# stm233/image-compression-for-machine

Measured on AMD Instinct MI355X. Metric: images/sec (256x256) cnn-hyperprior (WACNN) training step, higher is better.
Workload: dtype f32; 1 GPU; cnn (WACNN N=192 M=320) train step, lambda=0.0067 MSE, batch 16/GPU synthetic 256x256, Adam lr 1e-4 + aux Adam, clip 1.0; global_batch=16, parallelism=dp1

## Files before the change

image-compression-for-machine_amd/csrc/winattn_mfma.hip:

```cpp
#include "icm_common.h"

namespace icm {

struct WaDesc;

struct WmDesc {
  const float* qkv;
  const float* table;
  float* out;
  const float* dout;
  float* dqkv;
  float* dtable_ws;
  int N, C, H, W, heads, shift, nwx, nwy;
  float scale;
};

#define WM_WS 8
#define WM_T 64
#define WM_TS 65
#define WM_NTAB 225

__device__ __forceinline__ int wm_region(int s, int L, int shift) { return s < L - WM_WS ? 0 : (s < L - shift ? 1 : 2); }

__device__ __forceinline__ void wm_token(const WmDesc& d, int wy, int wx, int t, int& pix, int& lab) {
  const int r = t >> 3, c = t & 7;
  const int sy = wy * WM_WS + r, sx = wx * WM_WS + c;
  int oy = sy + d.shift, ox = sx + d.shift;
  if (oy >= d.H) oy -= d.H;
  if (ox >= d.W) ox -= d.W;
  pix = oy * d.W + ox;
  lab = d.shift > 0 ? wm_region(sy, d.H, d.shift) * 3 + wm_region(sx, d.W, d.shift) : 0;
}

__device__ __forceinline__ int wm_row(int r) { return (r & 3) + 8 * (r >> 2); }
__device__ __forceinline__ int wm_relidx(int i, int j) {
  return ((i >> 3) - (j >> 3) + WM_WS - 1) * (2 * WM_WS - 1) + ((i & 7) - (j & 7) + WM_WS - 1);
}

template <int HD>
__device__ __forceinline__ void wm_tok_tok(const float* __restrict__ rowT, const float* __restrict__ colT, int lane,
                                           f32x16 (&acc)[2][2]) {
  const int l31 = lane & 31, h = lane >> 5;
#pragma unroll
  for (int x = 0; x < 2; ++x)
#pragma unroll
    for (int y = 0; y < 2; ++y)
#pragma unroll
      for (int r = 0; r < 16; ++r) acc[x][y][r] = 0.0f;
#pragma unroll
  for (int ks = 0; ks < HD / 2; ++ks) {
    const int off = (2 * ks + h) * WM_TS + l31;
    const float a0 = rowT[off], a1 = rowT[off + 32], b0 = colT[off], b1 = colT[off + 32];
    acc[0][0] = __builtin_amdgcn_mfma_f32_32x32x2f32(a0, b0, acc[0][0], 0, 0, 0);
    acc[0][1] = __builtin_amdgcn_mfma_f32_32x32x2f32(a0, b1, acc[0][1], 0, 0, 0);
    acc[1][0] = __builtin_amdgcn_mfma_f32_32x32x2f32(a1, b0, acc[1][0], 0, 0, 0);
    acc[1][1] = __builtin_amdgcn_mfma_f32_32x32x2f32(a1, b1, acc[1][1], 0, 0, 0);
  }
}

template <int HD, int ND>
__device__ __forceinline__ void wm_ch_tok(const float* __restrict__ chT, const f32x16 (&M)[2][2], int lane,
                                          f32x16 (&o)[ND][2]) {
  const int l31 = lane & 31, h = lane >> 5;
#pragma unroll
  for (int dt = 0; dt < ND; ++dt)
#pragma unroll
    for (int y = 0; y < 2; ++y)
#pragma unroll
      for (int r = 0; r < 16; ++r) o[dt][y][r] = 0.0f;
#pragma unroll
  for (int x = 0; x < 2; ++x)
#pragma unroll
    for (int r = 0; r < 16; ++r) {
      const int tok = x * 32 + wm_row(r) + 4 * h;
#pragma unroll
      for (int dt = 0; dt < ND; ++dt) {
        const int dd = min(dt * 32 + l31, HD - 1);
        const float a = chT[dd * WM_TS + tok];
        o[dt][0] = __builtin_amdgcn_mfma_f32_32x32x2f32(a, M[x][0][r], o[dt][0], 0, 0, 0);
        o[dt][1] = __builtin_amdgcn_mfma_f32_32x32x2f32(a, M[x][1][r], o[dt][1], 0, 0, 0);
      }
    }
}

template <int HD, int ND>
__device__ __forceinline__ void wm_store(float* __restrict__ base, long long HW, const int (&pix)[2], int lane,
                                         const f32x16 (&o)[ND][2], float mul) {
  const int h = lane >> 5;
#pragma unroll
  for (int dt = 0; dt < ND; ++dt)
#pragma unroll
    for (int r = 0; r < 16; ++r) {
      const int dd = dt * 32 + wm_row(r) + 4 * h;
      if (dd < HD) {
        base[(long long)dd * HW + pix[0]] = o[dt][0][r] * mul;
        base[(long long)dd * HW + pix[1]] = o[dt][1][r] * mul;
      }
    }
}

template <int HD, int NS>
__device__ __forceinline__ void wm_load_all(const float* const (&src)[NS], long long HW, int pix, int lane, float mul0,
                                            float* __restrict__ dst0) {
  float v[NS][HD];
#pragma unroll
  for (int k = 0; k < NS; ++k)
#pragma unroll
    for (int dd = 0; dd < HD; ++dd) v[k][dd] = src[k][(long long)dd * HW + pix];
#pragma unroll
  for (int k = 0; k < NS; ++k)
#pragma unroll
    for (int dd = 0; dd < HD; ++dd) dst0[(k * HD + dd) * WM_TS + lane] = k == 0 ? v[k][dd] * mul0 : v[k][dd];
}

__device__ __forceinline__ float wm_xhalf(float v) { return __shfl_xor(v, 32, 64); }

__device__ __forceinline__ void wm_softmax_T(f32x16 (&acc)[2][2], const float* __restrict__ bias, const int (&labq)[2],
                                             const unsigned char* __restrict__ labs, bool masked, int lane,
                                             float (&m)[2], float (&linv)[2]) {
  const int l31 = lane & 31, h = lane >> 5;
#pragma unroll
  for (int it = 0; it < 2; ++it) {
    const int i = it * 32 + l31;
    float mx = -3.0e38f;
#pragma unroll
    for (int jt = 0; jt < 2; ++jt)
#pragma unroll
      for (int r = 0; r < 16; ++r) {
        const int j = jt * 32 + wm_row(r) + 4 * h;
        float s = acc[jt][it][r] + bias[wm_relidx(i, j)];
        if (masked && labs[j] != labq[it]) s += -100.0f;
        acc[jt][it][r] = s;
        mx = fmaxf(mx, s);
      }
    mx = fmaxf(mx, wm_xhalf(mx));
    float sum = 0.0f;
#pragma unroll
    for (int jt = 0; jt < 2; ++jt)
#pragma unroll
      for (int r = 0; r < 16; ++r) {
        const float p = expf(acc[jt][it][r] - mx);
        acc[jt][it][r] = p;
        sum += p;
      }
    sum += wm_xhalf(sum);
    const float inv = 1.0f / sum;
#pragma unroll
    for (int jt = 0; jt < 2; ++jt)
#pragma unroll
      for (int r = 0; r < 16; ++r) acc[jt][it][r] *= inv;
    m[it] = mx;
    linv[it] = inv;
  }
}

template <int HD, int NS>
struct WmLds {
  static constexpr int kSlab = HD * WM_TS;
  static constexpr int kFloats = NS * kSlab + 228 + (NS > 3 ? 228 + 3 * WM_T : 0);
};

template <int HD>
__global__ __launch_bounds__(256, 2) void winattn_mfma_fwd_kernel(const WmDesc d) {
  extern __shared__ __attribute__((aligned(16))) float smem[];
  constexpr int ND = (HD + 31) / 32;
  using LDS = WmLds<HD, 3>;
  int* pixs = reinterpret_cast<int*>(smem + 4 * LDS::kFloats);
  unsigned char* labs = reinterpret_cast<unsigned char*>(pixs + WM_T);
  const int tid = threadIdx.x, lane = tid & 63, wave = __builtin_amdgcn_readfirstlane(tid >> 6);
  float* Qt = smem + wave * LDS::kFloats;
  float* Kt = Qt + LDS::kSlab;
  float* Vt = Kt + LDS::kSlab;
  float* bias = Vt + LDS::kSlab;
  int bid = xcd_block_id();
  const int wx = bid % d.nwx; bid /= d.nwx;
  const int wy = bid % d.nwy;
  const int n = bid / d.nwy;
  const long long HW = (long long)d.H * d.W;
  if (tid < WM_T) {
    int px, lb;
    wm_token(d, wy, wx, tid, px, lb);
    pixs[tid] = px;
    labs[tid] = (unsigned char)lb;
  }
  __syncthreads();
  const int l31 = lane & 31;
  const int mypix = pixs[lane];
  const int pix2[2] = {pixs[l31], pixs[32 + l31]};
  const int labq[2] = {labs[l31], labs[32 + l31]};
  const float* base = d.qkv + (long long)n * 3 * d.C * HW;
  const bool masked = d.shift > 0;
  for (int head = wave; head < d.heads; head += 4) {
    {
      const float* const srcs[3] = {base + (long long)(head * HD) * HW, base + (long long)(d.C + head * HD) * HW,
                                    base + (long long)(2 * d.C + head * HD) * HW};
      wm_load_all<HD, 3>(srcs, HW, mypix, lane, d.scale, Qt);
    }
    for (int e = lane; e < WM_NTAB; e += 64) bias[e] = d.table[e * d.heads + head];
    __builtin_amdgcn_s_waitcnt(0);
    __builtin_amdgcn_wave_barrier();
    f32x16 st[2][2];
    wm_tok_tok<HD>(Kt, Qt, lane, st);
    float m[2], linv[2];
    wm_softmax_T(st, bias, labq, labs, masked, lane, m, linv);
    f32x16 o[ND][2];
    wm_ch_tok<HD, ND>(Vt, st, lane, o);
    wm_store<HD, ND>(d.out + ((long long)n * d.C + head * HD) * HW, HW, pix2, lane, o, 1.0f);
    __builtin_amdgcn_s_waitcnt(0);
    __builtin_amdgcn_wave_barrier();
  }
}

template <int HD>
__global__ __launch_bounds__(256, 1) void winattn_mfma_bwd_kernel(const WmDesc d) {
  extern __shared__ __attribute__((aligned(16))) float smem[];
  constexpr int ND = (HD + 31) / 32;
  using LDS = WmLds<HD, 4>;
  int* pixs = reinterpret_cast<int*>(smem + 4 * LDS::kFloats);
  unsigned char* labs = reinterpret_cast<unsigned char*>(pixs + WM_T);
  const int tid = threadIdx.x, lane = tid & 63, wave = __builtin_amdgcn_readfirstlane(tid >> 6);
  float* Qt = smem + wave * LDS::kFloats;
  float* Kt = Qt + LDS::kSlab;
  float* Vt = Kt + LDS::kSlab;
  float* Gt = Vt + LDS::kSlab;
  float* bias = Gt + LDS::kSlab;
  float* dbias = bias + 228;
  float* stat_m = dbias + 228;
  float* stat_l = stat_m + WM_T;
  float* stat_d = stat_l + WM_T;
  int bid = xcd_block_id();
  const int win = bid;
  const int wx = bid % d.nwx; bid /= d.nwx;
  const int wy = bid % d.nwy;
  const int n = bid / d.nwy;
  const long long HW = (long long)d.H * d.W;
  if (tid < WM_T) {
    int px, lb;
    wm_token(d, wy, wx, tid, px, lb);
    pixs[tid] = px;
    labs[tid] = (unsigned char)lb;
  }
  __syncthreads();
  const int l31 = lane & 31, h = lane >> 5;
  const int mypix = pixs[lane];
  const int pix2[2] = {pixs[l31], pixs[32 + l31]};
  const int labq[2] = {labs[l31], labs[32 + l31]};
  const float* base = d.qkv + (long long)n * 3 * d.C * HW;
  float* dbase = d.dqkv + (long long)n * 3 * d.C * HW;
  const bool masked = d.shift > 0;
  for (int head = wave; head < d.heads; head += 4) {
    {
      const float* const srcs[4] = {base + (long long)(head * HD) * HW, base + (long long)(d.C + head * HD) * HW,
                                    base + (long long)(2 * d.C + head * HD) * HW,
                                    d.dout + ((long long)n * d.C + head * HD) * HW};
      wm_load_all<HD, 4>(srcs, HW, mypix, lane, d.scale, Qt);
    }
    for (int e = lane; e < WM_NTAB; e += 64) {
      bias[e] = d.table[e * d.heads + head];
      dbias[e] = 0.0f;
    }
    __builtin_amdgcn_s_waitcnt(0);
    __builtin_amdgcn_wave_barrier();
    {
      f32x16 pt[2][2];
      wm_tok_tok<HD>(Kt, Qt, lane, pt);
      float m[2], linv[2];
      wm_softmax_T(pt, bias, labq, labs, masked, lane, m, linv);
      if (h == 0) {
        stat_m[l31] = m[0]; stat_m[32 + l31] = m[1];
        stat_l[l31] = linv[0]; stat_l[32 + l31] = linv[1];
      }
      f32x16 dpt[2][2];
      wm_tok_tok<HD>(Vt, Gt, lane, dpt);
#pragma unroll
      for (int it = 0; it < 2; ++it) {
        float del = 0.0f;
#pragma unroll
        for (int jt = 0; jt < 2; ++jt)
#pragma unroll
          for (int r = 0; r < 16; ++r) del += pt[jt][it][r] * dpt[jt][it][r];
        del += wm_xhalf(del);
        if (h == 0) stat_d[it * 32 + l31] = del;
#pragma unroll
        for (int jt = 0; jt < 2; ++jt)
#pragma unroll
          for (int r = 0; r < 16; ++r) pt[jt][it][r] *= dpt[jt][it][r] - del;
      }
#pragma unroll
      for (int hh = 0; hh < 2; ++hh) {
        if (h == hh) {
#pragma unroll
          for (int it = 0; it < 2; ++it)
#pragma unroll
            for (int jt = 0; jt < 2; ++jt)
#pragma unroll
              for (int r = 0; r < 16; ++r) {
                const int idx = wm_relidx(it * 32 + l31, jt * 32 + wm_row(r) + 4 * h);
                __hip_atomic_fetch_add(dbias + idx, pt[jt][it][r], __ATOMIC_RELAXED, __HIP_MEMORY_SCOPE_WAVEFRONT);
              }
        }
        __builtin_amdgcn_s_waitcnt(0);
        __builtin_amdgcn_wave_barrier();
      }
      f32x16 o[ND][2];
      wm_ch_tok<HD, ND>(Kt, pt, lane, o);
      wm_store<HD, ND>(dbase + (long long)(head * HD) * HW, HW, pix2, lane, o, d.scale);
    }
    __builtin_amdgcn_s_waitcnt(0);
    __builtin_amdgcn_wave_barrier();
    {
      f32x16 p[2][2];
      wm_tok_tok<HD>(Qt, Kt, lane, p);
#pragma unroll
      for (int it = 0; it < 2; ++it)
#pragma unroll
        for (int r = 0; r < 16; ++r) {
          const int i = it * 32 + wm_row(r) + 4 * h;
          const float mi = stat_m[i], li = stat_l[i];
          const int labi = labs[i];
#pragma unroll
          for (int jt = 0; jt < 2; ++jt) {
            const int j = jt * 32 + l31;
            float s = p[it][jt][r] + bias[wm_relidx(i, j)];
            if (masked && labq[jt] != labi) s += -100.0f;
            p[it][jt][r] = expf(s - mi) * li;
          }
        }
      {
        f32x16 o[ND][2];
        wm_ch_tok<HD, ND>(Gt, p, lane, o);
        wm_store<HD, ND>(dbase + (long long)(2 * d.C + head * HD) * HW, HW, pix2, lane, o, 1.0f);
      }
      f32x16 dp[2][2];
      wm_tok_tok<HD>(Gt, Vt, lane, dp);
#pragma unroll
      for (int it = 0; it < 2; ++it)
#pragma unroll
        for (int r = 0; r < 16; ++r) {
          const float del = stat_d[it * 32 + wm_row(r) + 4 * h];
#pragma unroll
          for (int jt = 0; jt < 2; ++jt) p[it][jt][r] *= dp[it][jt][r] - del;
        }
      f32x16 o[ND][2];
      wm_ch_tok<HD, ND>(Qt, p, lane, o);
      wm_store<HD, ND>(dbase + (long long)(d.C + head * HD) * HW, HW, pix2, lane, o, 1.0f);
    }
    {
      float* slab = d.dtable_ws + ((long long)win * d.heads + head) * WM_NTAB;
      for (int e = lane; e < WM_NTAB; e += 64) slab[e] = dbias[e];
    }
    __builtin_amdgcn_s_waitcnt(0);
    __builtin_amdgcn_wave_barrier();
  }
}

typedef void (*WmFn)(const WmDesc);
static bool wm_pick(int hd, WmFn& f, WmFn& b, size_t& lf, size_t& lb) {
  switch (hd) {
#define C_(n)                                               \
  case n:                                                   \
    f = winattn_mfma_fwd_kernel<n>;                         \
    b = winattn_mfma_bwd_kernel<n>;                         \
    lf = ((size_t)4 * WmLds<n, 3>::kFloats + WM_T + WM_T / 4) * sizeof(float);  \
    lb = ((size_t)4 * WmLds<n, 4>::kFloats + WM_T + WM_T / 4) * sizeof(float);  \
    return true;
    C_(8) C_(16) C_(24) C_(32) C_(48)
#undef C_
    default: return false;
  }
}

static bool wm_fill(WmDesc& d, int N, int C, int H, int W, int heads, int ws, int shift) {
  if (ws != WM_WS || heads <= 0 || C % heads || H % ws || W % ws || shift < 0 || shift >= ws) return false;
  d.N = N; d.C = C; d.H = H; d.W = W; d.heads = heads; d.shift = shift;
  d.nwx = W / ws; d.nwy = H / ws;
  d.scale = 1.0f / sqrtf((float)(C / heads));
  return true;
}

int winattn_mfma_fwd(const float* qkv, const float* table, float* out, int N, int C, int H, int W, int heads, int ws,
                     int shift, hipStream_t stream) {
  WmDesc d{};
  WmFn f, b;
  size_t lf, lb;
  if (!wm_fill(d, N, C, H, W, heads, ws, shift) || !wm_pick(C / heads, f, b, lf, lb)) return -1;
  d.qkv = qkv; d.table = table; d.out = out;
  if (lf > 64 * 1024 && !ensure_max_lds(reinterpret_cast<const void*>(f))) return ICM_ERR_LAUNCH;
  hipLaunchKernelGGL(f, dim3(N * d.nwy * d.nwx), dim3(256), lf, stream, d);
  ICM_CHECK_LAUNCH();
  return ICM_OK;
}

int winattn_mfma_bwd(const float* qkv, const float* table, const float* dout, float* dqkv, float* dtable_ws, int N, int C,
                     int H, int W, int heads, int ws, int shift, hipStream_t stream) {
  WmDesc d{};
  WmFn f, b;
  size_t lf, lb;
  if (!wm_fill(d, N, C, H, W, heads, ws, shift) || !wm_pick(C / heads, f, b, lf, lb)) return -1;
  d.qkv = qkv; d.table = table; d.dout = dout; d.dqkv = dqkv; d.dtable_ws = dtable_ws;
  if (lb > 160 * 1024) return -1;
  if (lb > 64 * 1024 && !ensure_max_lds(reinterpret_cast<const void*>(b))) return ICM_ERR_LAUNCH;
  hipLaunchKernelGGL(b, dim3(N * d.nwy * d.nwx), dim3(256), lb, stream, d);
  ICM_CHECK_LAUNCH();
  return ICM_OK;
}

}

namespace icm {

#define W4_T 16
#define W4_TS 17
#define W4_NTAB 49

struct W4Desc {
  const float* qkv;
  const float* table;
  float* out;
  const float* dout;
  float* dqkv;
  float* dtable_ws;
  int N, C, H, W, heads, shift, ngx, nwy;
  float scale;
};

typedef float f32x4v __attribute__((ext_vector_type(4)));

__device__ __forceinline__ int w4_region(int s, int L, int shift) { return s < L - 4 ? 0 : (s < L - shift ? 1 : 2); }

template <int HD>
__device__ __forceinline__ f32x4v w4_tok_tok(const float* __restrict__ rowT, const float* __restrict__ colT, int lane) {
  const int t = lane & 15, g = lane >> 4;
  f32x4v acc = {0.0f, 0.0f, 0.0f, 0.0f};
#pragma unroll
  for (int ks = 0; ks < HD / 4; ++ks) {
    const int off = (4 * ks + g) * W4_TS + t;
    acc = __builtin_amdgcn_mfma_f32_16x16x4f32(rowT[off], colT[off], acc, 0, 0, 0);
  }
  return acc;
}
template <int HD, int ND>
__device__ __forceinline__ void w4_ch_tok(const float* __restrict__ chT, const f32x4v M, int lane, f32x4v (&o)[ND]) {
  const int t = lane & 15, g = lane >> 4;
#pragma unroll
  for (int dt = 0; dt < ND; ++dt) {
    o[dt] = f32x4v{0.0f, 0.0f, 0.0f, 0.0f};
    const int dd = min(dt * 16 + t, HD - 1);
#pragma unroll
    for (int r = 0; r < 4; ++r)
      o[dt] = __builtin_amdgcn_mfma_f32_16x16x4f32(chT[dd * W4_TS + 4 * g + r], M[r], o[dt], 0, 0, 0);
  }
}
template <int HD, int ND>
__device__ __forceinline__ void w4_store(float* __restrict__ base, long long HW, int pix, int lane, const f32x4v (&o)[ND],
                                         float mul) {
  const int g = lane >> 4;
#pragma unroll
  for (int dt = 0; dt < ND; ++dt)
#pragma unroll
    for (int r = 0; r < 4; ++r) {
      const int dd = dt * 16 + 4 * g + r;
      if (dd < HD) base[(long long)dd * HW + pix] = o[dt][r] * mul;
    }
}
__device__ __forceinline__ float w4_xgroups(float v, bool is_max) {
  const float a = __shfl_xor(v, 16, 64);
  v = is_max ? fmaxf(v, a) : v + a;
  const float b = __shfl_xor(v, 32, 64);
  return is_max ? fmaxf(v, b) : v + b;
}
__device__ __forceinline__ int w4_relidx(int i, int j) { return ((i >> 2) - (j >> 2) + 3) * 7 + ((i & 3) - (j & 3) + 3); }

template <int HD, int NS>
struct W4Lds {
  static constexpr int kSlab = HD * W4_TS;
  static constexpr int kFloats = NS * 4 * kSlab + 52 + (NS > 3 ? 52 + 3 * 64 : 0);
};

template <int HD, int NS>
__device__ __forceinline__ void w4_load_all(const float* const (&src)[NS], long long HW, int pix, int lane, float mul0,
                                            float* __restrict__ dst0) {
  const int w = lane >> 4, t = lane & 15;
  float v[NS][HD];
#pragma unroll
  for (int k = 0; k < NS; ++k)
#pragma unroll
    for (int dd = 0; dd < HD; ++dd) v[k][dd] = src[k][(long long)dd * HW + pix];
#pragma unroll
  for (int k = 0; k < NS; ++k)
#pragma unroll
    for (int dd = 0; dd < HD; ++dd)
      dst0[((k * 4 + w) * HD + dd) * W4_TS + t] = k == 0 ? v[k][dd] * mul0 : v[k][dd];
}

__device__ __forceinline__ void w4_token(const W4Desc& d, int wy, int gx, int w, int t, int& pix, int& lab, bool& valid) {
  const int wx = gx * 4 + w;
  valid = wx * 4 < d.W;
  const int r = t >> 2, c = t & 3;
  const int sy = wy * 4 + r, sx = min(wx, d.W / 4 - 1) * 4 + c;
  int oy = sy + d.shift, ox = sx + d.shift;
  if (oy >= d.H) oy -= d.H;
  if (ox >= d.W) ox -= d.W;
  pix = oy * d.W + ox;
  lab = d.shift > 0 ? w4_region(sy, d.H, d.shift) * 3 + w4_region(sx, d.W, d.shift) : 0;
}

template <int HD>
__global__ __launch_bounds__(256) void winattn_mfma16_fwd_kernel(const W4Desc d) {
  extern __shared__ __attribute__((aligned(16))) float smem[];
  constexpr int ND = (HD + 15) / 16;
  using LDS = W4Lds<HD, 3>;
  const int tid = threadIdx.x, lane = tid & 63, wave = __builtin_amdgcn_readfirstlane(tid >> 6);
  float* slabs = smem + wave * LDS::kFloats;
  float* bias = slabs + 3 * 4 * LDS::kSlab;
  const int wt = blockIdx.x * 4 + wave;
  const int ntask = d.N * d.nwy * d.ngx;
  if (wt >= ntask * d.heads) return;
  const int head = wt % d.heads, task = wt / d.heads;
  const int gx = task % d.ngx;
  const int wy = (task / d.ngx) % d.nwy;
  const int n = task / (d.ngx * d.nwy);
  const long long HW = (long long)d.H * d.W;
  const int t = lane & 15, g = lane >> 4;
  int mypix, mylab;
  bool myvalid;
  w4_token(d, wy, gx, g, t, mypix, mylab, myvalid);
  const float* base = d.qkv + (long long)n * 3 * d.C * HW;
  const bool masked = d.shift > 0;
  {
    {
      const float* const srcs[3] = {base + (long long)(head * HD) * HW, base + (long long)(d.C + head * HD) * HW,
                                    base + (long long)(2 * d.C + head * HD) * HW};
      w4_load_all<HD, 3>(srcs, HW, mypix, lane, d.scale, slabs);
    }
    if (lane < W4_NTAB) bias[lane] = d.table[lane * d.heads + head];
    __builtin_amdgcn_s_waitcnt(0);
    __builtin_amdgcn_wave_barrier();
#pragma unroll 1
    for (int w = 0; w < 4; ++w) {
      int pixw, labq;
      bool validw;
      w4_token(d, wy, gx, w, t, pixw, labq, validw);
      if (!validw) break;
      const float* Qt = slabs + (0 * 4 + w) * LDS::kSlab;
      const float* Kt = slabs + (1 * 4 + w) * LDS::kSlab;
      const float* Vt = slabs + (2 * 4 + w) * LDS::kSlab;
      f32x4v st = w4_tok_tok<HD>(Kt, Qt, lane);
      float mx = -3.0e38f;
#pragma unroll
      for (int r = 0; r < 4; ++r) {
        const int j = 4 * g + r;
        float s = st[r] + bias[w4_relidx(t, j)];
        if (masked) {
          int pj, lj; bool vj;
          w4_token(d, wy, gx, w, j, pj, lj, vj);
          if (lj != labq) s += -100.0f;
        }
        st[r] = s;
        mx = fmaxf(mx, s);
      }
      mx = w4_xgroups(mx, true);
      float sum = 0.0f;
#pragma unroll
      for (int r = 0; r < 4; ++r) { st[r] = expf(st[r] - mx); sum += st[r]; }
      sum = w4_xgroups(sum, false);
      const float inv = 1.0f / sum;
#pragma unroll
      for (int r = 0; r < 4; ++r) st[r] *= inv;
      f32x4v o[ND];
      w4_ch_tok<HD, ND>(Vt, st, lane, o);
      w4_store<HD, ND>(d.out + ((long long)n * d.C + head * HD) * HW, HW, pixw, lane, o, 1.0f);
    }
    __builtin_amdgcn_s_waitcnt(0);
    __builtin_amdgcn_wave_barrier();
  }
}

template <int HD>
__global__ __launch_bounds__(128) void winattn_mfma16_bwd_kernel(const W4Desc d) {
  extern __shared__ __attribute__((aligned(16))) float smem[];
  constexpr int ND = (HD + 15) / 16;
  using LDS = W4Lds<HD, 4>;
  const int tid = threadIdx.x, lane = tid & 63, wave = __builtin_amdgcn_readfirstlane(tid >> 6);
  float* slabs = smem + wave * LDS::kFloats;
  float* bias = slabs + 4 * 4 * LDS::kSlab;
  float* dbias = bias + 52;
  float* stat_m = dbias + 52;
  float* stat_l = stat_m + 64;
  float* stat_d = stat_l + 64;
  const int wt = blockIdx.x * 2 + wave;
  const int ntask = d.N * d.nwy * d.ngx;
  if (wt >= ntask * d.heads) return;
  const int head = wt % d.heads, task = wt / d.heads;
  const int gx = task % d.ngx;
  const int wy = (task / d.ngx) % d.nwy;
  const int n = task / (d.ngx * d.nwy);
  const long long HW = (long long)d.H * d.W;
  const int t = lane & 15, g = lane >> 4;
  int mypix, mylab;
  bool myvalid;
  w4_token(d, wy, gx, g, t, mypix, mylab, myvalid);
  const float* base = d.qkv + (long long)n * 3 * d.C * HW;
  float* dbase = d.dqkv + (long long)n * 3 * d.C * HW;
  const bool masked = d.shift > 0;
  {
    {
      const float* const srcs[4] = {base + (long long)(head * HD) * HW, base + (long long)(d.C + head * HD) * HW,
                                    base + (long long)(2 * d.C + head * HD) * HW,
                                    d.dout + ((long long)n * d.C + head * HD) * HW};
      w4_load_all<HD, 4>(srcs, HW, mypix, lane, d.scale, slabs);
    }
    if (lane < W4_NTAB) { bias[lane] = d.table[lane * d.heads + head]; dbias[lane] = 0.0f; }
    __builtin_amdgcn_s_waitcnt(0);
    __builtin_amdgcn_wave_barrier();
#pragma unroll 1
    for (int w = 0; w < 4; ++w) {
      int pixw, labq;
      bool validw;
      w4_token(d, wy, gx, w, t, pixw, labq, validw);
      if (!validw) break;
      const float* Qt = slabs + (0 * 4 + w) * LDS::kSlab;
      const float* Kt = slabs + (1 * 4 + w) * LDS::kSlab;
      const float* Vt = slabs + (2 * 4 + w) * LDS::kSlab;
      const float* Gt = slabs + (3 * 4 + w) * LDS::kSlab;
      int labr[4];
#pragma unroll
      for (int r = 0; r < 4; ++r) {
        int pj; bool vj;
        w4_token(d, wy, gx, w, 4 * g + r, pj, labr[r], vj);
      }
      {
        f32x4v pt = w4_tok_tok<HD>(Kt, Qt, lane);
        float mx = -3.0e38f;
#pragma unroll
        for (int r = 0; r < 4; ++r) {
          float s = pt[r] + bias[w4_relidx(t, 4 * g + r)];
          if (masked && labr[r] != labq) s += -100.0f;
          pt[r] = s;
          mx = fmaxf(mx, s);
        }
        mx = w4_xgroups(mx, true);
        float sum = 0.0f;
#pragma unroll
        for (int r = 0; r < 4; ++r) { pt[r] = expf(pt[r] - mx); sum += pt[r]; }
        sum = w4_xgroups(sum, false);
        const float inv = 1.0f / sum;
        const f32x4v dpt = w4_tok_tok<HD>(Vt, Gt, lane);
        float del = 0.0f;
#pragma unroll
        for (int r = 0; r < 4; ++r) { pt[r] *= inv; del += pt[r] * dpt[r]; }
        del = w4_xgroups(del, false);
        if (g == 0) { stat_m[w * 16 + t] = mx; stat_l[w * 16 + t] = inv; stat_d[w * 16 + t] = del; }
#pragma unroll
        for (int r = 0; r < 4; ++r) pt[r] *= dpt[r] - del;
#pragma unroll
        for (int gg = 0; gg < 4; ++gg) {
          if (g == gg) {
#pragma unroll
            for (int r = 0; r < 4; ++r)
              __hip_atomic_fetch_add(dbias + w4_relidx(t, 4 * g + r), pt[r], __ATOMIC_RELAXED, __HIP_MEMORY_SCOPE_WAVEFRONT);
          }
          __builtin_amdgcn_s_waitcnt(0);
          __builtin_amdgcn_wave_barrier();
        }
        f32x4v o[ND];
        w4_ch_tok<HD, ND>(Kt, pt, lane, o);
        w4_store<HD, ND>(dbase + (long long)(head * HD) * HW, HW, pixw, lane, o, d.scale);
      }
      __builtin_amdgcn_s_waitcnt(0);
      __builtin_amdgcn_wave_barrier();
      {
        f32x4v p = w4_tok_tok<HD>(Qt, Kt, lane);
#pragma unroll
        for (int r = 0; r < 4; ++r) {
          const int i = 4 * g + r;
          float s = p[r] + bias[w4_relidx(i, t)];
          if (masked && labr[r] != labq) s += -100.0f;
          p[r] = expf(s - stat_m[w * 16 + i]) * stat_l[w * 16 + i];
        }
        {
          f32x4v o[ND];
          w4_ch_tok<HD, ND>(Gt, p, lane, o);
          w4_store<HD, ND>(dbase + (long long)(2 * d.C + head * HD) * HW, HW, pixw, lane, o, 1.0f);
        }
        const f32x4v dp = w4_tok_tok<HD>(Gt, Vt, lane);
#pragma unroll
        for (int r = 0; r < 4; ++r) p[r] *= dp[r] - stat_d[w * 16 + 4 * g + r];
        f32x4v o[ND];
        w4_ch_tok<HD, ND>(Qt, p, lane, o);
        w4_store<HD, ND>(dbase + (long long)(d.C + head * HD) * HW, HW, pixw, lane, o, 1.0f);
      }
    }
    if (lane < W4_NTAB) d.dtable_ws[((long long)task * d.heads + head) * W4_NTAB + lane] = dbias[lane];
    __builtin_amdgcn_s_waitcnt(0);
    __builtin_amdgcn_wave_barrier();
  }
}

typedef void (*W4Fn)(const W4Desc);
static bool w4_pick(int hd, W4Fn& f, W4Fn& b, size_t& lf, size_t& lb) {
  switch (hd) {
#define C_(n)                                                 \
  case n:                                                     \
    f = winattn_mfma16_fwd_kernel<n>;                         \
    b = winattn_mfma16_bwd_kernel<n>;                         \
    lf = (size_t)4 * W4Lds<n, 3>::kFloats * sizeof(float);    \
    lb = (size_t)2 * W4Lds<n, 4>::kFloats * sizeof(float);    \
    return true;
    C_(8) C_(16) C_(24) C_(32) C_(40)
#undef C_
    default: return false;
  }
}
static bool w4_fill(W4Desc& d, int N, int C, int H, int W, int heads, int ws, int shift) {
  if (ws != 4 || heads <= 0 || C % heads || H % 4 || W % 4 || shift < 0 || shift >= 4) return false;
  d.N = N; d.C = C; d.H = H; d.W = W; d.heads = heads; d.shift = shift;
  d.ngx = (W / 4 + 3) / 4; d.nwy = H / 4;
  d.scale = 1.0f / sqrtf((float)(C / heads));
  return true;
}

int winattn_mfma16_slabs(int N, int C, int H, int W, int heads, int ws, int shift) {
  W4Desc d{};
  W4Fn f, b;
  size_t lf, lb;
  if (!w4_fill(d, N, C, H, W, heads, ws, shift) || !w4_pick(C / heads, f, b, lf, lb) || lb > 160 * 1024) return -1;
  return N * d.nwy * d.ngx;
}

int winattn_mfma16_fwd(const float* qkv, const float* table, float* out, int N, int C, int H, int W, int heads, int ws,
                       int shift, hipStream_t stream) {
  W4Desc d{};
  W4Fn f, b;
  size_t lf, lb;
  if (!w4_fill(d, N, C, H, W, heads, ws, shift) || !w4_pick(C / heads, f, b, lf, lb) || lf > 160 * 1024) return -1;
  d.qkv = qkv; d.table = table; d.out = out;
  if (lf > 64 * 1024 && !ensure_max_lds(reinterpret_cast<const void*>(f))) return ICM_ERR_LAUNCH;
  const int nwt = N * d.nwy * d.ngx * heads;
  hipLaunchKernelGGL(f, dim3((nwt + 3) / 4), dim3(256), lf, stream, d);
  ICM_CHECK_LAUNCH();
  return ICM_OK;
}
int winattn_mfma16_bwd(const float* qkv, const float* table, const float* dout, float* dqkv, float* dtable_ws, int N,
                       int C, int H, int W, int heads, int ws, int shift, hipStream_t stream) {
  W4Desc d{};
  W4Fn f, b;
  size_t lf, lb;
  if (!w4_fill(d, N, C, H, W, heads, ws, shift) || !w4_pick(C / heads, f, b, lf, lb) || lb > 160 * 1024) return -1;
  d.qkv = qkv; d.table = table; d.dout = dout; d.dqkv = dqkv; d.dtable_ws = dtable_ws;
  if (lb > 64 * 1024 && !ensure_max_lds(reinterpret_cast<const void*>(b))) return ICM_ERR_LAUNCH;
  const int nwt = N * d.nwy * d.ngx * heads;
  hipLaunchKernelGGL(b, dim3((nwt + 1) / 2), dim3(128), lb, stream, d);
  ICM_CHECK_LAUNCH();
  return ICM_OK;
}

}
```

Baseline: 384.7 images/s.

## Split window-attention backward across wave pairs per head with vectorized staging

Measured after the change: 391.1 images/s, median of 6. +1.7%, better.

```diff
diff --git a/image-compression-for-machine_amd/csrc/winattn_mfma.hip b/image-compression-for-machine_amd/csrc/winattn_mfma.hip
--- a/image-compression-for-machine_amd/csrc/winattn_mfma.hip
+++ b/image-compression-for-machine_amd/csrc/winattn_mfma.hip
@@ -13,6 +13,7 @@
   float* dtable_ws;
   int N, C, H, W, heads, shift, nwx, nwy;
   float scale;
+  int vec;
 };
 
 #define WM_WS 8
@@ -157,7 +158,7 @@
 template <int HD, int NS>
 struct WmLds {
   static constexpr int kSlab = HD * WM_TS;
-  static constexpr int kFloats = NS * kSlab + 228 + (NS > 3 ? 228 + 3 * WM_T : 0);
+  static constexpr int kFloats = NS * kSlab + 228;
 };
 
 template <int HD>
@@ -212,22 +213,115 @@
 }
 
 template <int HD>
-__global__ __launch_bounds__(256, 1) void winattn_mfma_bwd_kernel(const WmDesc d) {
+struct WpLds {
+  static constexpr int kSlab = HD * WM_TS;
+  static constexpr int kFloats = 4 * kSlab + 228 + 2 * 228 + 3 * WM_T;
+  static constexpr size_t kBytes = ((size_t)4 * kFloats + WM_T + WM_T / 4) * sizeof(float);
+};
+
+template <int HD>
+__device__ __forceinline__ void wp_tok_tok(const float* __restrict__ rowT, const float* __restrict__ colT, int ct,
+                                           int lane, f32x16 (&acc)[2]) {
+  const int l31 = lane & 31, h = lane >> 5;
+#pragma unroll
+  for (int x = 0; x < 2; ++x)
+#pragma unroll
+    for (int r = 0; r < 16; ++r) acc[x][r] = 0.0f;
+#pragma unroll
+  for (int ks = 0; ks < HD / 2; ++ks) {
+    const int off = (2 * ks + h) * WM_TS + l31;
+    const float a0 = rowT[off], a1 = rowT[off + 32], b = colT[off + 32 * ct];
+    acc[0] = __builtin_amdgcn_mfma_f32_32x32x2f32(a0, b, acc[0], 0, 0, 0);
+    acc[1] = __builtin_amdgcn_mfma_f32_32x32x2f32(a1, b, acc[1], 0, 0, 0);
+  }
+}
+
+template <int HD, int ND>
+__device__ __forceinline__ void wp_ch_tok(const float* __restrict__ chT, const f32x16 (&M)[2], int lane,
+                                          f32x16 (&o)[ND]) {
+  const int l31 = lane & 31, h = lane >> 5;
+#pragma unroll
+  for (int dt = 0; dt < ND; ++dt)
+#pragma unroll
+    for (int r = 0; r < 16; ++r) o[dt][r] = 0.0f;
+#pragma unroll
+  for (int x = 0; x < 2; ++x)
+#pragma unroll
+    for (int r = 0; r < 16; ++r) {
+      const int tok = x * 32 + wm_row(r) + 4 * h;
+#pragma unroll
+      for (int dt = 0; dt < ND; ++dt) {
+        const int dd = min(dt * 32 + l31, HD - 1);
+        o[dt] = __builtin_amdgcn_mfma_f32_32x32x2f32(chT[dd * WM_TS + tok], M[x][r], o[dt], 0, 0, 0);
+      }
+    }
+}
+
+template <int HD, int ND>
+__device__ __forceinline__ void wp_store(float* __restrict__ base, long long HW, int pix, int lane,
+                                         const f32x16 (&o)[ND], float mul) {
+  const int h = lane >> 5;
+#pragma unroll
+  for (int dt = 0; dt < ND; ++dt)
+#pragma unroll
+    for (int r = 0; r < 16; ++r) {
+      const int dd = dt * 32 + wm_row(r) + 4 * h;
+      if (dd < HD) base[(long long)dd * HW + pix] = o[dt][r] * mul;
+    }
+}
+
+template <int HD>
+__device__ __forceinline__ void wp_stage_vec(const float* __restrict__ src0, const float* __restrict__ src1,
+                                             long long HW, int pix4, int lane, float mul0, float* __restrict__ dst) {
+  const int g4 = lane & 15, rsub = lane >> 4;
+  f32x4 v[HD / 2];
+#pragma unroll
+  for (int k = 0; k < HD / 2; ++k) {
+    const int row = 4 * k + rsub, s = (4 * k) / HD, dd = row - s * HD;
+    v[k] = *reinterpret_cast<const f32x4*>((s ? src1 : src0) + (long long)dd * HW + pix4);
+  }
+#pragma unroll
+  for (int k = 0; k < HD / 2; ++k) {
+    const int row = 4 * k + rsub;
+    float* o = dst + row * WM_TS + 4 * g4;
+    if ((4 * k) / HD == 0) v[k] *= mul0;
+    o[0] = v[k][0]; o[1] = v[k][1]; o[2] = v[k][2]; o[3] = v[k][3];
+  }
+}
+template <int HD>
+__device__ __forceinline__ void wp_stage_dword(const float* __restrict__ src0, const float* __restrict__ src1,
+                                               long long HW, int pix, int lane, float mul0, float* __restrict__ dst) {
+  float v[2][HD];
+#pragma unroll
+  for (int k = 0; k < 2; ++k)
+#pragma unroll
+    for (int dd = 0; dd < HD; ++dd) v[k][dd] = (k ? src1 : src0)[(long long)dd * HW + pix];
+#pragma unroll
+  for (int k = 0; k < 2; ++k)
+#pragma unroll
+    for (int dd = 0; dd < HD; ++dd) dst[(k * HD + dd) * WM_TS + lane] = k == 0 ? v[k][dd] * mul0 : v[k][dd];
+}
+
+template <int HD>
+__global__ __launch_bounds__(512) void winattn_mfma_bwd_pair_kernel(const WmDesc d) {
   extern __shared__ __attribute__((aligned(16))) float smem[];
   constexpr int ND = (HD + 31) / 32;
-  using LDS = WmLds<HD, 4>;
+  using LDS = WpLds<HD>;
   int* pixs = reinterpret_cast<int*>(smem + 4 * LDS::kFloats);
   unsigned char* labs = reinterpret_cast<unsigned char*>(pixs + WM_T);
   const int tid = threadIdx.x, lane = tid & 63, wave = __builtin_amdgcn_readfirstlane(tid >> 6);
-  float* Qt = smem + wave * LDS::kFloats;
+  const int pair = wave >> 1, w = wave & 1;
+  float* Qt = smem + pair * LDS::kFloats;
   float* Kt = Qt + LDS::kSlab;
   float* Vt = Kt + LDS::kSlab;
   float* Gt = Vt + LDS::kSlab;
   float* bias = Gt + LDS::kSlab;
-  float* dbias = bias + 228;
-  float* stat_m = dbias + 228;
+  float* dbias0 = bias + 228;
+  float* dbias1 = dbias0 + 228;
+  float* stat_m = dbias1 + 228;
   float* stat_l = stat_m + WM_T;
   float* stat_d = stat_l + WM_T;
+  float* dbias = w ? dbias1 : dbias0;
   int bid = xcd_block_id();
   const int win = bid;
   const int wx = bid % d.nwx; bid /= d.nwx;
@@ -242,75 +336,99 @@
   }
   __syncthreads();
   const int l31 = lane & 31, h = lane >> 5;
-  const int mypix = pixs[lane];
-  const int pix2[2] = {pixs[l31], pixs[32 + l31]};
-  const int labq[2] = {labs[l31], labs[32 + l31]};
+  const int ctok = w * 32 + l31;
+  const int cpix = pixs[ctok], clab = labs[ctok];
+  const int spix = d.vec ? pixs[4 * (lane & 15)] : pixs[lane];
   const float* base = d.qkv + (long long)n * 3 * d.C * HW;
   float* dbase = d.dqkv + (long long)n * 3 * d.C * HW;
-  const bool masked = d.shift > 0;
-  for (int head = wave; head < d.heads; head += 4) {
-    {
-      const float* const srcs[4] = {base + (long long)(head * HD) * HW, base + (long long)(d.C + head * HD) * HW,
-                                    base + (long long)(2 * d.C + head * HD) * HW,
-                                    d.dout + ((long long)n * d.C + head * HD) * HW};
-      wm_load_all<HD, 4>(srcs, HW, mypix, lane, d.scale, Qt);
-    }
-    for (int e = lane; e < WM_NTAB; e += 64) {
-      bias[e] = d.table[e * d.heads + head];
-      dbias[e] = 0.0f;
-    }
-    __builtin_amdgcn_s_waitcnt(0);
-    __builtin_amdgcn_wave_barrier();
-    {
-      f32x16 pt[2][2];
-      wm_tok_tok<HD>(Kt, Qt, lane, pt);
-      float m[2], linv[2];
-      wm_softmax_T(pt, bias, labq, labs, masked, lane, m, linv);
+  const int rounds = (d.heads + 3) >> 2;
+  for (int rd = 0; rd < rounds; ++rd) {
+    const int head = rd * 4 + pair;
+    const bool active = head < d.heads;
+    if (active) {
+      const float* src0 = w ? base + (long long)(2 * d.C + head * HD) * HW : base + (long long)(head * HD) * HW;
+      const float* src1 = w ? d.dout + ((long long)n * d.C + head * HD) * HW
+                            : base + (long long)(d.C + head * HD) * HW;
+      const float mul0 = w ? 1.0f : d.scale;
+      if (d.vec) wp_stage_vec<HD>(src0, src1, HW, spix, lane, mul0, Qt + w * 2 * LDS::kSlab);
+      else wp_stage_dword<HD>(src0, src1, HW, spix, lane, mul0, Qt + w * 2 * LDS::kSlab);
+      for (int e = w * 64 + lane; e < WM_NTAB; e += 128) {
+        bias[e] = d.table[e * d.heads + head];
+        dbias0[e] = 0.0f;
+        dbias1[e] = 0.0f;
+      }
+    }
+    __syncthreads();
+    if (active) {
+      f32x16 pt[2];
+      wp_tok_tok<HD>(Kt, Qt, w, lane, pt);
+      float mx = -3.0e38f;
+#pragma unroll
+      for (int jt = 0; jt < 2; ++jt)
+#pragma unroll
+        for (int r = 0; r < 16; ++r) {
+          const int j = jt * 32 + wm_row(r) + 4 * h;
+          float s = pt[jt][r] + bias[wm_relidx(ctok, j)];
+          if (labs[j] != clab) s += -100.0f;
+          pt[jt][r] = s;
+          mx = fmaxf(mx, s);
+        }
+      mx = fmaxf(mx, wm_xhalf(mx));
+      float sum = 0.0f;
+#pragma unroll
+      for (int jt = 0; jt < 2; ++jt)
+#pragma unroll
+        for (int r = 0; r < 16; ++r) {
+          const float p = expf(pt[jt][r] - mx);
+          pt[jt][r] = p;
+          sum += p;
+        }
+      sum += wm_xhalf(sum);
+      const float inv = 1.0f / sum;
+#pragma unroll
+      for (int jt = 0; jt < 2; ++jt)
+#pragma unroll
+        for (int r = 0; r < 16; ++r) pt[jt][r] *= inv;
+      f32x16 dpt[2];
+      wp_tok_tok<HD>(Vt, Gt, w, lane, dpt);
+      float del = 0.0f;
+#pragma unroll
+      for (int jt = 0; jt < 2; ++jt)
+#pragma unroll
+        for (int r = 0; r < 16; ++r) del += pt[jt][r] * dpt[jt][r];
+      del += wm_xhalf(del);
       if (h == 0) {
-        stat_m[l31] = m[0]; stat_m[32 + l31] = m[1];
-        stat_l[l31] = linv[0]; stat_l[32 + l31] = linv[1];
-      }
-      f32x16 dpt[2][2];
-      wm_tok_tok<HD>(Vt, Gt, lane, dpt);
-#pragma unroll
-      for (int it = 0; it < 2; ++it) {
-        float del = 0.0f;
+        stat_m[ctok] = mx;
+        stat_l[ctok] = inv;
+        stat_d[ctok] = del;
+      }
+#pragma unroll
+      for (int jt = 0; jt < 2; ++jt)
+#pragma unroll
+        for (int r = 0; r < 16; ++r) pt[jt][r] *= dpt[jt][r] - del;
+      {
+        volatile float* tb = dbias;
 #pragma unroll
         for (int jt = 0; jt < 2; ++jt)
 #pragma unroll
-          for (int r = 0; r < 16; ++r) del += pt[jt][it][r] * dpt[jt][it][r];
-        del += wm_xhalf(del);
-        if (h == 0) stat_d[it * 32 + l31] = del;
-#pragma unroll
-        for (int jt = 0; jt < 2; ++jt)
-#pragma unroll
-          for (int r = 0; r < 16; ++r) pt[jt][it][r] *= dpt[jt][it][r] - del;
-      }
-#pragma unroll
-      for (int hh = 0; hh < 2; ++hh) {
-        if (h == hh) {
-#pragma unroll
-          for (int it = 0; it < 2; ++it)
-#pragma unroll
-            for (int jt = 0; jt < 2; ++jt)
-#pragma unroll
-              for (int r = 0; r < 16; ++r) {
-                const int idx = wm_relidx(it * 32 + l31, jt * 32 + wm_row(r) + 4 * h);
-                __hip_atomic_fetch_add(dbias + idx, pt[jt][it][r], __ATOMIC_RELAXED, __HIP_MEMORY_SCOPE_WAVEFRONT);
-              }
-        }
-        __builtin_amdgcn_s_waitcnt(0);
-        __builtin_amdgcn_wave_barrier();
-      }
-      f32x16 o[ND][2];
-      wm_ch_tok<HD, ND>(Kt, pt, lane, o);
-      wm_store<HD, ND>(dbase + (long long)(head * HD) * HW, HW, pix2, lane, o, d.scale);
-    }
-    __builtin_amdgcn_s_waitcnt(0);
-    __builtin_amdgcn_wave_barrier();
-    {
-      f32x16 p[2][2];
-      wm_tok_tok<HD>(Qt, Kt, lane, p);
+          for (int r = 0; r < 16; ++r) {
+            const float x = h ? pt[jt ^ 1][r] : pt[jt][r];
+            const int idx = wm_relidx(ctok, (jt ^ h) * 32 + wm_row(r) + 4 * h);
+            tb[idx] = tb[idx] + x;
+          }
+      }
+      f32x16 o[ND];
+      wp_ch_tok<HD, ND>(Kt, pt, lane, o);
+      wp_store<HD, ND>(dbase + (long long)(head * HD) * HW, HW, cpix, lane, o, d.scale);
+    }
+    __syncthreads();
+    if (active) {
+      {
+        float* slab = d.dtable_ws + ((long long)win * d.heads + head) * WM_NTAB;
+        for (int e = w * 64 + lane; e < WM_NTAB; e += 128) slab[e] = dbias0[e] + dbias1[e];
+      }
+      f32x16 p[2];
+      wp_tok_tok<HD>(Qt, Kt, w, lane, p);
 #pragma unroll
       for (int it = 0; it < 2; ++it)
 #pragma unroll
@@ -318,53 +436,50 @@
           const int i = it * 32 + wm_row(r) + 4 * h;
           const float mi = stat_m[i], li = stat_l[i];
           const int labi = labs[i];
-#pragma unroll
-          for (int jt = 0; jt < 2; ++jt) {
-            const int j = jt * 32 + l31;
-            float s = p[it][jt][r] + bias[wm_relidx(i, j)];
-            if (masked && labq[jt] != labi) s += -100.0f;
-            p[it][jt][r] = expf(s - mi) * li;
-          }
+          float s = p[it][r] + bias[wm_relidx(i, ctok)];
+          if (clab != labi) s += -100.0f;
+          p[it][r] = expf(s - mi) * li;
         }
       {
-        f32x16 o[ND][2];
-        wm_ch_tok<HD, ND>(Gt, p, lane, o);
-        wm_store<HD, ND>(dbase + (long long)(2 * d.C + head * HD) * HW, HW, pix2, lane, o, 1.0f);
-      }
-      f32x16 dp[2][2];
-      wm_tok_tok<HD>(Gt, Vt, lane, dp);
+        f32x16 o[ND];
+        wp_ch_tok<HD, ND>(Gt, p, lane, o);
+        wp_store<HD, ND>(dbase + (long long)(2 * d.C + head * HD) * HW, HW, cpix, lane, o, 1.0f);
+      }
+      f32x16 dp[2];
+      wp_tok_tok<HD>(Gt, Vt, w, lane, dp);
 #pragma unroll
       for (int it = 0; it < 2; ++it)
 #pragma unroll
-        for (int r = 0; r < 16; ++r) {
-          const float del = stat_d[it * 32 + wm_row(r) + 4 * h];
-#pragma unroll
-          for (int jt = 0; jt < 2; ++jt) p[it][jt][r] *= dp[it][jt][r] - del;
-        }
-      f32x16 o[ND][2];
-      wm_ch_tok<HD, ND>(Qt, p, lane, o);
-      wm_store<HD, ND>(dbase + (long long)(d.C + head * HD) * HW, HW, pix2, lane, o, 1.0f);
-    }
-    {
-      float* slab = d.dtable_ws + ((long long)win * d.heads + head) * WM_NTAB;
-      for (int e = lane; e < WM_NTAB; e += 64) slab[e] = dbias[e];
-    }
-    __builtin_amdgcn_s_waitcnt(0);
-    __builtin_amdgcn_wave_barrier();
+        for (int r = 0; r < 16; ++r) p[it][r] *= dp[it][r] - stat_d[it * 32 + wm_row(r) + 4 * h];
+      f32x16 o[ND];
+      wp_ch_tok<HD, ND>(Qt, p, lane, o);
+      wp_store<HD, ND>(dbase + (long long)(d.C + head * HD) * HW, HW, cpix, lane, o, 1.0f);
+    }
+    __syncthreads();
   }
 }
 
 typedef void (*WmFn)(const WmDesc);
-static bool wm_pick(int hd, WmFn& f, WmFn& b, size_t& lf, size_t& lb) {
+static bool wm_pick_fwd(int hd, WmFn& f, size_t& lf) {
   switch (hd) {
 #define C_(n)                                               \
   case n:                                                   \
     f = winattn_mfma_fwd_kernel<n>;                         \
-    b = winattn_mfma_bwd_kernel<n>;                         \
     lf = ((size_t)4 * WmLds<n, 3>::kFloats + WM_T + WM_T / 4) * sizeof(float);  \
-    lb = ((size_t)4 * WmLds<n, 4>::kFloats + WM_T + WM_T / 4) * sizeof(float);  \
     return true;
     C_(8) C_(16) C_(24) C_(32) C_(48)
+#undef C_
+    default: return false;
+  }
+}
+static bool wm_pick_bwd(int hd, WmFn& b, size_t& lb) {
+  switch (hd) {
+#define C_(n)                                 \
+  case n:                                     \
+    b = winattn_mfma_bwd_pair_kernel<n>;      \
+    lb = WpLds<n>::kBytes;                    \
+    return true;
+    C_(8) C_(16) C_(24) C_(32)
 #undef C_
     default: return false;
   }
@@ -381,9 +496,9 @@
 int winattn_mfma_fwd(const float* qkv, const float* table, float* out, int N, int C, int H, int W, int heads, int ws,
                      int shift, hipStream_t stream) {
   WmDesc d{};
-  WmFn f, b;
-  size_t lf, lb;
-  if (!wm_fill(d, N, C, H, W, heads, ws, shift) || !wm_pick(C / heads, f, b, lf, lb)) return -1;
+  WmFn f;
+  size_t lf;
+  if (!wm_fill(d, N, C, H, W, heads, ws, shift) || !wm_pick_fwd(C / heads, f, lf)) return -1;
   d.qkv = qkv; d.table = table; d.out = out;
   if (lf > 64 * 1024 && !ensure_max_lds(reinterpret_cast<const void*>(f))) return ICM_ERR_LAUNCH;
   hipLaunchKernelGGL(f, dim3(N * d.nwy * d.nwx), dim3(256), lf, stream, d);
@@ -394,13 +509,14 @@
 int winattn_mfma_bwd(const float* qkv, const float* table, const float* dout, float* dqkv, float* dtable_ws, int N, int C,
                      int H, int W, int heads, int ws, int shift, hipStream_t stream) {
   WmDesc d{};
-  WmFn f, b;
-  size_t lf, lb;
-  if (!wm_fill(d, N, C, H, W, heads, ws, shift) || !wm_pick(C / heads, f, b, lf, lb)) return -1;
+  WmFn b;
+  size_t lb;
+  if (!wm_fill(d, N, C, H, W, heads, ws, shift) || !wm_pick_bwd(C / heads, b, lb)) return -1;
   d.qkv = qkv; d.table = table; d.dout = dout; d.dqkv = dqkv; d.dtable_ws = dtable_ws;
+  d.vec = shift % 4 == 0 && (reinterpret_cast<uintptr_t>(qkv) | reinterpret_cast<uintptr_t>(dout)) % 16 == 0;
   if (lb > 160 * 1024) return -1;
   if (lb > 64 * 1024 && !ensure_max_lds(reinterpret_cast<const void*>(b))) return ICM_ERR_LAUNCH;
-  hipLaunchKernelGGL(b, dim3(N * d.nwy * d.nwx), dim3(256), lb, stream, d);
+  hipLaunchKernelGGL(b, dim3(N * d.nwy * d.nwx), dim3(512), lb, stream, d);
   ICM_CHECK_LAUNCH();
   return ICM_OK;
 }
```
